# davnords/octic-vits

Measured on AMD Instinct MI355X. Metric: images/sec Hybrid Octic ViT-H/14 224² bf16 train step @1/2/4/8 MI355X, higher is better.
Workload: dtype bf16; 1 GPU; hybrid_deit_huge_patch14 (16 octic + 16 standard blocks, drop_path 0.5) DeiT-III train step: bf16-autocast fwd + bwd + LAMB + EMA, 224x224, batch 64/GPU (BASELINE configs[1]), data parallel over 1 GPU(s); global_batch=64, per_gpu_batch=64, accum_steps=1, parallelism=dp1, library_gemm_table=True, launch=hipGraph replay (whole step)

## Files before the change

include/octic_hip.h:

```cpp
#ifndef OCTIC_HIP_H
#define OCTIC_HIP_H

#include <stdint.h>

#ifdef __cplusplus
extern "C" {
#endif

#define OCTIC_ABI_VERSION 20

enum { OCTIC_F32 = 0, OCTIC_BF16 = 1, OCTIC_U8 = 2  };

enum {
  OCTIC_OK = 0,
  OCTIC_ESHAPE = -1,
  OCTIC_EALIGN = -2,
  OCTIC_EDTYPE = -3,
  OCTIC_ENULL = -4,
  OCTIC_EWORKSPACE = -5
};

typedef struct {
  void* ptr[5];
  int64_t ld[5];
// ... 47 lines not shown
  int c;
} octic_ln_finish_job;
int octic_layernorm_d8_bwd_finish_batch(const octic_ln_finish_job* jobs, int njobs, void* stream);

int octic_sample_blocks(const void* src, void* dst, const int64_t* idx, int64_t n, int64_t block_bytes, int scatter,
                        void* stream);

int octic_linear_d8_fwd(const octic_view* x, const void* const w[5], const float* bias, const octic_view* y,
                        const octic_view* resid, const float* rs, int64_t rows_per_sample,
                        const float* const cs[5], int64_t M, int cin, int cout, int dtype, int out_dtype,
                        void* stream);
int octic_linear_d8_fwd_skip(const octic_view* x, const void* const w[5], const float* bias, const octic_view* y,
                             const octic_view* resid, const float* rs, int64_t rows_per_sample,
                             const float* const cs[5], int64_t M, int cin, int cout, int dtype, int out_dtype,
                             const float* sample_scale, int64_t skip_rows_per_sample, void* stream);

int octic_linear_d8_prep(const float* const w32[5], const float* const cs[5], int cin, int cout, void* wb, void* wt,
                         int dtype, void* stream);
typedef struct octic_prep_item {
  const float* w[5];
  const float* cs[5];
  void* wb;
  void* wt;
  int32_t cin, cout;
  int32_t block_begin, block_count;
} octic_prep_item;
int octic_linear_d8_prep_batch_blocks(int cin, int cout);
int octic_linear_d8_prep_batch(const octic_prep_item* items_dev, int n_items, int total_blocks, int dtype, void* stream);

int octic_linear_d8_tile_n(int64_t M, int cin, int cout);
enum {
  OCTIC_LINEAR_WREG = 0,
  OCTIC_LINEAR_RING = 1,
  OCTIC_LINEAR_CLASSIC = 2
};
int octic_linear_d8_plan(int64_t M, int cin, int cout, int dtype, int out_dtype, int fused, int out[4]);
int octic_linear_d8_ring_order(int ngroups, const int* items, const int* ksteps, int slots_per_xcd, int* out_group,
                               int* out_item);

int octic_linear_d8_wgrad_has_colsum(int cin, int cout, int dtype);
enum {
  OCTIC_WGRAD_RING = 0,
  OCTIC_WGRAD_TILED = 1
};
int octic_linear_d8_wgrad_plan(int64_t M, int cin, int cout, int dtype, int out[4]);
int64_t octic_linear_d8_wgrad_workspace_bytes(int cin, int cout, int splits);
int octic_linear_d8_wgrad_splits(int64_t M, int cin, int cout);
int octic_linear_d8_wgrad_tile(int64_t M, int cin, int cout);
int octic_linear_d8_wgrad(const octic_view* x, const octic_view* dy, int64_t M, int cin, int cout, int dtype,
                          float* workspace, int splits, void* stream);
int octic_linear_d8_wgrad_finish(const float* workspace, int splits, int cin, int cout,
                                 const float* const w32[5], const float* const cs[5], const float* bias,
                                 const float* dysum, float* const dw[5], float* const dcs[5], float* dbias,
// ... 266 lines not shown
```

octic_vits_amd/_lib.py:

```python
import ctypes
import os
import re

HERE = os.path.dirname(os.path.abspath(__file__))
LIB_PATH = os.environ.get("OCTIC_LIB") or os.path.join(HERE, "liboctic_hip.so")
HEADER_PATH = os.path.join(HERE, "..", "include", "octic_hip.h")

F32, BF16, U8 = 0, 1, 2
ABI_VERSION = 20
(ROUTE_DENSE_TILE, ROUTE_DENSE_SPLIT, ROUTE_WGRAD_SLABS, ROUTE_WGRAD_TILE, ROUTE_LINEAR_RING, ROUTE_RING_EVEN,
 ROUTE_ATTN_LEGACY, ROUTE_ATTN_ONLINE, ROUTE_ATTN_BWD_PAIR, ROUTE_DENSE_IMAGE, ROUTE_DENSE_CLS2, ROUTE_ATTN_STREAM) = range(12)

(ATTN_FWD_PERSIST, ATTN_FWD_A80_ONESHOT, ATTN_FWD_A80_ONLINE, ATTN_FWD_RESIDENT, ATTN_FWD_STREAM, ATTN_FWD_F32) = range(6)
ATTN_BWD_SINGLE, ATTN_BWD_PAIR, ATTN_BWD_STREAM, ATTN_BWD_F32 = range(4)
LINEAR_WREG, LINEAR_RING, LINEAR_CLASSIC = range(3)
WGRAD_RING, WGRAD_TILED = range(2)

c_i64, c_int, c_float, c_void_p = ctypes.c_int64, ctypes.c_int, ctypes.c_float, ctypes.c_void_p
c_double = ctypes.c_double


class OcticView(ctypes.Structure):
    _fields_ = [("ptr", c_void_p * 5), ("ld", c_i64 * 5)]

# ... 9 lines not shown
    "octic_gelu_d8_bwd": (c_int, [VP, VP, VP, c_i64, c_int, c_int, c_void_p]),
    "octic_gelu_d8_fwd_skip": (c_int, [VP, VP, c_i64, c_int, c_int, c_void_p, c_i64, c_void_p]),
    "octic_gelu_d8_bwd_skip": (c_int, [VP, VP, VP, c_i64, c_int, c_int, c_void_p, c_i64, c_void_p]),
    "octic_layernorm_d8_fwd": (c_int, [VP, VP, c_void_p, c_void_p, c_void_p, c_i64, c_int, c_float, c_int, c_void_p]),
    "octic_layernorm_d8_bwd_blocks": (c_int, [c_i64]),
    "octic_layernorm_d8_bwd": (c_int, [VP, VP, c_void_p, c_void_p, VP, VP, c_void_p, c_i64, c_int, c_int, c_void_p]),
    "octic_layernorm_d8_bwd_cast": (c_int, [VP, VP, c_void_p, c_void_p, VP, VP, c_void_p, c_i64, c_int, c_void_p, c_i64,
                                            c_void_p, c_void_p]),
    "octic_layernorm_d8_bwd_finish": (c_int, [c_void_p, c_int, c_int, c_void_p, c_void_p, c_void_p]),
    "octic_layernorm_d8_bwd_finish_batch": (c_int, [c_void_p, c_int, c_void_p]),
    "octic_sample_blocks": (c_int, [c_void_p, c_void_p, c_void_p, c_i64, c_i64, c_int, c_void_p]),
    "octic_linear_d8_fwd": (c_int, [VP, c_void_p, c_void_p, VP, VP, c_void_p, c_i64, c_void_p, c_i64, c_int, c_int,
                                    c_int, c_int, c_void_p]),
    "octic_linear_d8_fwd_skip": (c_int, [VP, c_void_p, c_void_p, VP, VP, c_void_p, c_i64, c_void_p, c_i64, c_int, c_int,
                                         c_int, c_int, c_void_p, c_i64, c_void_p]),
    "octic_linear_d8_tile_n": (c_int, [c_i64, c_int, c_int]),
    "octic_linear_d8_plan": (c_int, [c_i64, c_int, c_int, c_int, c_int, c_int, ctypes.POINTER(c_int)]),
    "octic_linear_d8_ring_order": (c_int, [c_void_p, c_void_p, c_void_p, c_int, c_void_p, c_void_p]),
    "octic_linear_d8_wgrad_tile": (c_int, [c_i64, c_int, c_int]),
    "octic_linear_d8_wgrad_workspace_bytes": (c_i64, [c_int, c_int, c_int]),
    "octic_linear_d8_wgrad_splits": (c_int, [c_i64, c_int, c_int]),
    "octic_linear_d8_wgrad": (c_int, [VP, VP, c_i64, c_int, c_int, c_int, c_void_p, c_int, c_void_p]),
    "octic_linear_d8_wgrad_finish": (c_int, [c_void_p, c_int, c_int, c_int, c_void_p, c_void_p, c_void_p, c_void_p,
                                             c_void_p, c_void_p, c_void_p, c_void_p]),
    "octic_linear_d8_wgrad_finish_batch": (c_int, [c_void_p, c_int, c_void_p]),
    "octic_linear_d8_wgrad_has_colsum": (c_int, [c_int, c_int, c_int]),
    "octic_linear_d8_wgrad_plan": (c_int, [c_i64, c_int, c_int, c_int, ctypes.POINTER(c_int)]),
    "octic_lamb_workspace_floats": (c_i64, [c_int, c_int]),
    "octic_lamb_step": (c_int, [c_void_p] * 10 + [c_int, c_int, c_void_p, c_float, c_float, c_float, c_float, c_float,
                                                  c_int, c_float, c_void_p, c_void_p]),
    "octic_adamw_step": (c_int, [c_void_p] * 10 + [c_int, c_int, c_void_p, c_float, c_float, c_float, c_float, c_float,
                                                   c_int, c_float, c_void_p, c_void_p]),
    "octic_lamb_step_hp": (c_int, [c_void_p] * 10 + [c_int, c_int, c_void_p, c_void_p, c_float, c_float, c_float, c_float,
# ... 185 lines not shown
```

octic_vits_amd/csrc/gemm.hip:

```cpp
#include <stdlib.h>
#include <type_traits>
#include <mutex>
#include <vector>
#include "gemm_args.hpp"

namespace octic {

template <typename T> struct Elem;
template <> struct Elem<float> { static constexpr int EPC = 4; typedef f32x4 frag; };
template <> struct Elem<bf16> { static constexpr int EPC = 8; typedef bf16x8 frag; };

template <typename TOUT>
__device__ inline void store_out4(TOUT* p, f32x4 v);
template <>
__device__ inline void store_out4<float>(float* p, f32x4 v) { *(f32x4*)p = v; }
template <>
__device__ inline void store_out4<bf16>(bf16* p, f32x4 v) {
  bf16x4 o = {(bf16)v[0], (bf16)v[1], (bf16)v[2], (bf16)v[3]};
  *(bf16x4*)p = o;
}
template <typename TOUT>
__device__ inline f32x4 load_out4(const TOUT* p);
template <>
__device__ inline f32x4 load_out4<float>(const float* p) { return *(const f32x4*)p; }
// ... 287 lines not shown
    int r = tile - cum(k);
    bool found = false;
#pragma unroll
    for (int i = 0; i < 5; ++i) {
      const int s0 = (int)(((int64_t)k * T[i]) >> 3), sz = (int)(((int64_t)(k + 1) * T[i]) >> 3) - s0;
      if (!found && r < sz) {
        gi = i;
        lt = s0 + r;
        found = true;
      }
      if (!found) r -= sz;
    }
  }
}

template <typename TIN, typename TOUT, int EPI, int NT, int S, int BM = 128>
__global__ __launch_bounds__(BM * 2, 2) void linear_d8_ring_kernel(GemmArgs args) {
  constexpr int NW = BM / 32;
  constexpr int EPC = Elem<TIN>::EPC;
  constexpr int BKE = 8 * EPC;
  constexpr int MT = 2;
  constexpr int BN = 16 * NT;
  constexpr int STAGE = (BM + BN) * 128;
  constexpr int WI = BN / 8;
  constexpr int WQ = (WI + NW - 1) / NW;
  typedef typename Elem<TIN>::frag frag;
  extern __shared__ __attribute__((aligned(16))) char lds[];

  const int nwg = gridDim.x, bid = blockIdx.x;
  const int xcd = bid & 7, q8 = nwg >> 3, r8 = nwg & 7;
  const int tile = (xcd < r8 ? xcd * (q8 + 1) : r8 * (q8 + 1) + (xcd - r8) * q8) + (bid >> 3);
  (void)tile;
  int gi, lt;
  ring_item_of(args, nwg, bid, gi, lt);
  const GemmGroup& G = args.g[gi];
  const int mt = lt / G.n_chunks, nc = lt - mt * G.n_chunks;
  const int64_t m0 = (int64_t)mt * BM;
  const int nt_begin = nc * G.chunk;
  const int nt_count = (G.n_tiles - nt_begin) < G.chunk ? (G.n_tiles - nt_begin) : G.chunk;
  const int K = G.K, N = G.N;
  const int nkt = (K + BKE - 1) / BKE;
  const int steps = nt_count * nkt;
  const bool last_half_only = (K - (nkt - 1) * BKE) <= 4 * EPC;

  const int lane = threadIdx.x & 63;
  const int wid = __builtin_amdgcn_readfirstlane(threadIdx.x >> 6);
  const int fr = lane & 15, kg = lane >> 4;
  RTRACE(0);
#ifdef OCTIC_RING_TRACE
  {
    unsigned xcc, hwid;
    asm volatile("s_getreg_b32 %0, hwreg(HW_REG_XCC_ID)" : "=s"(xcc));
    asm volatile("s_getreg_b32 %0, hwreg(HW_REG_HW_ID)" : "=s"(hwid));
    if (tile < 2048 && lane == 0 && wid < 4) g_ring_trace[(tile * 4 + wid) * 64 + 63] = ((unsigned long long)hwid << 32) | xcc;
  }
#endif

  const int drow = lane >> 3;
  const int dkc = (lane & 7) ^ drow;
  const char* xsrc[4];
#pragma unroll
  for (int q = 0; q < 4; ++q) {
    int64_t mm = m0 + wid * 32 + q * 8 + drow;
    mm = mm < G.rows ? mm : G.rows - 1;
    const int64_t off = G.pair ? (mm >> 1) * G.a_ld + (mm & 1) * (int64_t)K : mm * G.a_ld;
    xsrc[q] = G.a + off * (int64_t)sizeof(TIN);
  }
  const int w_rem = WI % NW;
  const int w_cnt = WI / NW + (wid < w_rem ? 1 : 0);
  const int w_first = wid * (WI / NW) + (wid < w_rem ? wid : w_rem);
  const int dma_cnt = 4 + w_cnt;
// ... 325 lines not shown
    a.g[i].chunk = 1;
    a.g[i].n_chunks = a.g[i].n_tiles;
    a.g[i].tile_begin = t;
    t += a.g[i].n_chunks * a.g[i].m_tiles;
  }
  a.total_tiles = t;
  const size_t smem = (size_t)S * (BM + BN) * 128;
  {
    const int per_cu = (int)(160 * 1024 / smem) < 2 ? (int)(160 * 1024 / smem) : 2;
    plan_ring(a, t, device_cus() / 8 * (per_cu > 0 ? per_cu : 1));
  }
  static DeviceOnce once;
  if (once.first()) {
    (void)hipFuncSetAttribute((const void*)linear_d8_ring_kernel<TIN, TOUT, 0, NT, S, BM>, hipFuncAttributeMaxDynamicSharedMemorySize, (int)smem);
    (void)hipFuncSetAttribute((const void*)linear_d8_ring_kernel<TIN, TOUT, 1, NT, S, BM>, hipFuncAttributeMaxDynamicSharedMemorySize, (int)smem);
    (void)hipGetLastError();
  }
  if (fused) linear_d8_ring_kernel<TIN, TOUT, 1, NT, S, BM><<<t, BM * 2, smem, s>>>(a);
  else linear_d8_ring_kernel<TIN, TOUT, 0, NT, S, BM><<<t, BM * 2, smem, s>>>(a);
  return launch_status();
}

inline bool ring_ok(const GemmArgs& a, int dtype) {
  const int kstep = dtype == OCTIC_BF16 ? 32 : 16;
  for (int i = 0; i < a.ngroups; ++i)
    if (a.g[i].K % kstep) return false;
  return true;
}

inline bool ring_wide(const GemmArgs& a, int dtype) {
  bool ok = dtype == OCTIC_BF16 && a.lift_np == 0;
// ... 112 lines not shown
  for (int g = 0; g < ngroups; ++g) {
    a.g[g].K = ksteps[g] * 64;
    a.g[g].n_chunks = 1;
    a.g[g].chunk = 1;
    a.g[g].n_tiles = 1;
    a.g[g].m_tiles = items[g];
    a.g[g].tile_begin = t;
    t += items[g];
  }
  a.total_tiles = t;
  plan_ring(a, t, slots_per_xcd);
  for (int bid = 0; bid < t; ++bid) ring_item_of(a, t, bid, out_group[bid], out_item[bid]);
  return a.plan_mode;
}

extern "C" {

int octic_linear_d8_fwd_skip(const octic_view* x, const void* const w[5], const float* bias, const octic_view* y,
                             const octic_view* resid, const float* rs, int64_t rows_per_sample, const float* const cs[5],
                             int64_t M, int cin, int cout, int dtype, int out_dtype, const float* sample_scale,
                             int64_t skip_rows_per_sample, void* stream) {
  int e;
  if (sample_scale && (resid || rs || cs || skip_rows_per_sample <= 0 || M % skip_rows_per_sample != 0)) return OCTIC_ESHAPE;
  if ((e = check_c_dt(cin, dtype)) || (e = check_c_dt(cout, dtype)) || (e = check_c_dt(cout, out_dtype))) return e;
  if ((e = check_view(x, cin, dtype)) || (e = check_view(y, cout, out_dtype))) return e;
  if (resid && (e = check_view(resid, cout, out_dtype))) return e;
  if (!w) return OCTIC_ENULL;
  for (int i = 0; i < 5; ++i)
    if (!w[i] || (((uintptr_t)w[i]) & 15)) return w[i] ? OCTIC_EALIGN : OCTIC_ENULL;
  if (M <= 0 || (rs && rows_per_sample <= 0)) return OCTIC_ESHAPE;
  if (cs)
    for (int i = 0; i < 5; ++i)
      if (!cs[i]) return OCTIC_ENULL;
  GemmArgs a = {};
  a.rs = rs;
  a.rps = rs ? rows_per_sample : 1;
  a.skip = sample_scale;
  a.skip_rps = sample_scale ? skip_rows_per_sample : 1;
  d8_group_table(a, M, cin, cout);
  for (int gidx = 0; gidx < 5; ++gidx) {
    const int irrep = d8_group_irrep(gidx);
    GemmGroup& g = a.g[gidx];
    g.a = (const char*)x->ptr[irrep];
    g.a_ld = x->ld[irrep];
    g.w = (const char*)w[irrep];
    g.y = (char*)y->ptr[irrep];
    g.y_ld = y->ld[irrep];
    g.resid = resid ? (const char*)resid->ptr[irrep] : nullptr;
    g.r_ld = resid ? resid->ld[irrep] : 0;
    g.bias = (irrep == 0) ? bias : nullptr;
    g.cs = cs ? cs[irrep] : nullptr;
  }
  return dispatch_gemm(a, dtype, out_dtype, (hipStream_t)stream);
}

int octic_linear_d8_fwd(const octic_view* x, const void* const w[5], const float* bias, const octic_view* y,
                        const octic_view* resid, const float* rs, int64_t rows_per_sample, const float* const cs[5],
                        int64_t M, int cin, int cout, int dtype, int out_dtype, void* stream) {
  return octic_linear_d8_fwd_skip(x, w, bias, y, resid, rs, rows_per_sample, cs, M, cin, cout, dtype, out_dtype, nullptr, 0, stream);
}

int octic_linear_d8_plan(int64_t M, int cin, int cout, int dtype, int out_dtype, int fused, int out[4]) {
  if (!out) return OCTIC_ENULL;
  int e;
  if ((e = check_c_dt(cin, dtype)) || (e = check_c_dt(cout, dtype)) || (e = check_c_dt(cout, out_dtype))) return e;
  if (M <= 0) return OCTIC_ESHAPE;
  GemmArgs a = {};
  d8_group_table(a, M, cin, cout);
// ... 45 lines not shown
```

octic_vits_amd/csrc/gemm_args.hpp:

```cpp
#pragma once
#include "octic_common.hpp"

namespace octic {

struct GemmGroup {
  const char* a;
  int64_t a_ld;
  const char* w;
  char* y;
  int64_t y_ld;
  const char* resid;
  int64_t r_ld;
  const float* bias;
  const float* cs;
  int64_t rows;
  int K, N;
  int pair;
  int n_tiles, m_tiles;
  int chunk, n_chunks;
  int tile_begin;
  int wgs;
};

struct GemmArgs {
  GemmGroup g[5];
  int ngroups;
  int total_tiles;
  const float* rs;
  int64_t rps;
  int64_t lift_np;
  int lift_tok0;
  int plan_mode;
  int plan_nshort;
  int plan_a[8], plan_e[8];
  int plan_eb[8], plan_sb[8];
  const float* skip;
  int64_t skip_rps;
};

__device__ __forceinline__ unsigned lds_addr(const void* p) { return (unsigned)(uintptr_t)(__attribute__((address_space(3))) const char*)p; }
__device__ __forceinline__ bf16x8 lds_read16(unsigned addr) {
  bf16x8 v;
  asm volatile("ds_read_b128 %0, %1" : "=v"(v) : "v"(addr) : "memory");
  return v;
}
template <int N>
__device__ __forceinline__ void landed(bf16x8& v) {
  asm volatile("s_waitcnt lgkmcnt(%1)" : "+v"(v) : "n"(N) : "memory");
}

bool wreg_ok(const GemmArgs& a);
int launch_wreg(GemmArgs& a, int out_dtype, bool fused, hipStream_t s);
// ... 3 lines not shown
```

octic_vits_amd/d8_layers.py:

```python
import collections.abc
import math
from itertools import repeat

import torch
import torch.nn as nn
import torch.nn.functional as F

from . import functional as OF
from .d8_utils import SQRT2, SQRT2_OVER_4, convert_5tuple_to_8tuple, convert_8tuple_to_5tuple, expand_lift_kernel, packed_lift_weight
from .functional import Octic, as_packed, compute_dtype


def _ntuple(n):
    def parse(x):
        if isinstance(x, collections.abc.Iterable) and not isinstance(x, str):
            return tuple(x)
        return tuple(repeat(x, n))
    return parse


to_2tuple = _ntuple(2)

drop_path_mask_source = None

# ... 204 lines not shown
        if input_channels % 8 != 0 or output_channels % 8 != 0:
            raise ValueError()
        self.bias = bias
        self.input_channels, self.output_channels = input_channels, output_channels
        ci, co = input_channels // 8, output_channels // 8
        self.lin_A1 = nn.Linear(ci, co, bias=bias)
        self.lin_A2 = nn.Linear(ci, co, bias=False)
        self.lin_B1 = nn.Linear(ci, co, bias=False)
        self.lin_B2 = nn.Linear(ci, co, bias=False)
        self.lin_E = nn.Linear(2 * ci, 2 * co, bias=False)
        self._prep = OF.WeightPrep()

    def weights(self):
        return tuple(getattr(self, "lin_" + n).weight for n in _IRREPS)

    def forward(self, x_batched, resid=None, rs=None, cs=None, next_norm=None, skip_out=None, skip_dx=None):
        assert len(x_batched) == 5, "Input should be a 5-tuple"
        xp, cin = as_packed(x_batched)
        if 8 * cin != self.input_channels:
            raise ValueError(f"LinearD8: expected {self.input_channels} channels, got {8 * cin}")
        cout = self.output_channels // 8
        dtype = compute_dtype(xp)
        rps = xp.shape[-2] if xp.dim() >= 2 else 1
        if rs is not None and rs.numel() == xp.numel() // xp.shape[-1] and rs.numel() != xp.shape[0]:
            rps = 1
        cs5 = (None,) * 5 if cs is None else tuple(cs)
        if torch.compiler.is_compiling():
            from . import dispatch as _D
            xq = xp if xp.dtype == dtype else xp.to(dtype)
            fl = self._prep.flat if dtype == torch.bfloat16 else None
            pwb, pwt = fl if fl is not None else (None, None)
            y = torch.ops.octic.linear_d8(xq, *self.weights(), self.lin_A1.bias, resid, rs, *cs5, cin, cout, rps, pwb, pwt)
            return Octic(y, cout) if next_norm is None else (Octic(y, cout), None)
        if (next_norm is not None and resid is not None and OF.OCTIC_NEXT_NORM and xp.is_cuda and dtype == torch.bfloat16
                and resid.dtype == torch.float32 and type(next_norm) is LayerNormD8):
            a, beta = next_norm.affine()
            y, yn = OF.LinearD8NormFn.apply(xp, *self.weights(), self.lin_A1.bias, resid, rs, *cs5, cin, cout, rps, dtype,
                                            self._prep, *a, beta, next_norm.eps, skip_dx)
            return Octic(y, cout), Octic(yn, cout)
        y = OF.LinearD8Fn.apply(xp, *self.weights(), self.lin_A1.bias, resid, rs, *cs5, cin, cout, rps, dtype, self._prep,
                                skip_out, skip_dx)
        return Octic(y, cout) if next_norm is None else (Octic(y, cout), None)

    def extra_repr(self) -> str:
        return f"in_features={self.input_channels}, out_features={self.output_channels}, bias={self.bias is not None}"


class AffineD8(nn.Module):

    def __init__(self, dim, bias=True):
        super().__init__()
        if dim % 8 != 0:
            raise ValueError()
        self.alpha_A1 = nn.Parameter(torch.ones(dim // 8))
        self.alpha_A2 = nn.Parameter(torch.ones(dim // 8))
        self.alpha_B1 = nn.Parameter(torch.ones(dim // 8))
# ... 75 lines not shown
        self.fc2 = LinearD8(hidden_features, out_features, bias=bias[1])
        self.drop2 = DropoutD8(drop_probs[1])

    def _sample_mask(self, xs, resid, rs):
        if not (OF.LINEAR_SKIP_DROPPED and rs is not None and resid is not None and not COMPACT_DROP_PATH
                and type(self.fc1) is LinearD8 and type(self.fc2) is LinearD8 and type(self.act) is TritonGeluD8
                and type(self.norm) is nn.Identity and not self.drop1.active and not self.drop2.active
                and isinstance(xs, Octic) and xs.packed.dim() == 3 and xs.packed.is_cuda):
            return None
        xp = xs.packed
        return OF.linear_skip_scale(rs, xp.shape[1], xp.shape[0] * xp.shape[1])

    def forward(self, xs, resid=None, rs=None, cs=None, next_norm=None):
        mask = self._sample_mask(xs, resid, rs)
        if mask is not None:
            h = self.fc1(xs, skip_out=mask)
            a = Octic(OF.GeluD8PackedFn.apply(h.packed, h.c, mask, h.packed.shape[1]), h.c)
            return self.fc2(a, resid=resid, rs=rs, cs=cs, next_norm=next_norm, skip_dx=mask)
        xs = self.norm(self.drop1(self.act(self.fc1(xs))))
        if self.drop2.active or resid is None:
            out = _tail(self.drop2(self.fc2(xs)), resid, rs, cs)
            return out if next_norm is None else (out, None)
        return self.fc2(xs, resid=resid, rs=rs, cs=cs, next_norm=next_norm)


def _tail(ys, resid, rs, cs):
    if resid is None:
        return ys
    yp, c = as_packed(ys)
    yp = yp.to(resid.dtype)
    if cs is not None:
# ... 236 lines not shown
        if not OF.ops.attn_packed_ok(T, c, H, compute_dtype(xp)):
            return None
        if OF.skip_scale(rs, B) is None or OF.linear_skip_scale(rs, T, B * T) is None:
            return None
        if not OF.ops.attn_skips_dropped(B, T, 8 * (c // H), ld=(3 * 8 * c, 8 * c, 3 * 8 * c)):
            return None
        return rs

    def forward(self, xs, resid=None, rs=None, cs=None, next_norm=None):
        xp, c = as_packed(xs)
        if xp.dim() != 3:
            raise ValueError("AttentionD8 expects [B, N, C] irreps")
        drop = self.attn_drop.p if self.training else 0.
        rag = OF.RAGGED
        gemm_mask = self._gemm_mask(xp, c, resid, rs, drop, rag)
        qkv = self.qkv(xs if isinstance(xs, Octic) else Octic(xp, c), skip_out=gemm_mask)
        if rag is not None and rag.matches(xp):
            from . import ragged as _R
            if not (OF.ATTN_PACKED and drop == 0. and qkv.packed.is_cuda
                    and all(OF.ops.attn_packed_ok(T, c, self.num_heads, qkv.packed.dtype) for _, T, _ in rag.sets)):
                raise RuntimeError("AttentionD8: a ragged row tensor needs the packed attention kernels (bf16, head_dim 80 / 64)")
            on = Octic(_R.AttnPackedRaggedFn.apply(qkv.packed, rag, self.num_heads, c, (8 * c // self.num_heads) ** -0.5), c)
        elif (OF.ATTN_PACKED and drop == 0. and qkv.packed.is_cuda
                and OF.ops.attn_packed_ok(qkv.packed.shape[1], c, self.num_heads, qkv.packed.dtype)):
            if torch.compiler.is_compiling():
                from . import dispatch as _D
                on = Octic(torch.ops.octic.attn_packed(qkv.packed, self.num_heads, c, (8 * c // self.num_heads) ** -0.5)[0], c)
            else:
                on = Octic(OF.AttnPackedFn.apply(qkv.packed, self.num_heads, c, (8 * c // self.num_heads) ** -0.5,
                                                 None if (COMPACT_DROP_PATH or resid is None) else rs), c)
        else:
# ... 168 lines not shown
```

octic_vits_amd/functional.py:

```python
import os

import torch

from . import ops


class Octic(tuple):

    def __new__(cls, packed: torch.Tensor, c: int):
        self = super().__new__(cls, ops.split_packed(packed, c))
        self.packed, self.c = packed, c
        return self


def as_packed(xs):
    if isinstance(xs, Octic):
        return xs.packed, xs.c
    if len(xs) != 5:
        raise AssertionError("Input should be a 5-tuple")
    c = xs[0].shape[-1]
    if xs[4].shape[-2:] != (2, 2 * c):
        raise ValueError(f"E irrep must be [..., 2, {2 * c}], got {tuple(xs[4].shape)}")
    return torch.cat([xs[0], xs[1], xs[2], xs[3], xs[4].flatten(-2)], dim=-1), c

# ... 180 lines not shown
        return self.items is not None and self._current_ptrs() != self._ptrs

    def run(self):
        if self.items is None:
            return
        ops.check(ops.lib().octic_linear_d8_prep_batch(ops._p(self.items), len(self.preps), self.total_blocks,
                                                       ops.dt_code(torch.bfloat16), ops._stream(self.items)))
        for p, (wb, wt), flat in zip(self.preps, self.bufs, self.flats):
            p.adopt(wb, wt, flat)


class LinearD8Fn(torch.autograd.Function):

    @staticmethod
    def forward(ctx, x, wA1, wA2, wB1, wB2, wE, bias, resid, rs, sA1, sA2, sB1, sB2, sE, cin, cout, rps, dtype, prep,
                skip_out=None, skip_dx=None):
        w5 = (wA1, wA2, wB1, wB2, wE)
        cs5 = None if sA1 is None else (sA1, sA2, sB1, sB2, sE)
        ops._require_cuda(x)
        fused = resid is not None
        out_dtype = resid.dtype if fused else dtype
        x_in_dtype = x.dtype
        if x.dtype != dtype:
            x = ops.cast_rowscale(_c(x.float()), None, 1, dtype, cin)
        x = _c(x)
        wb, wt = prep.get(w5, cs5, dtype, cin, cout)
        lead = x.shape[:-1]
        M = x.numel() // (8 * cin)
        y = torch.empty(lead + (8 * cout,), dtype=out_dtype, device=x.device)
        b32 = None if bias is None else _c(bias.detach().float())
        cs32 = None if cs5 is None else [_c(s.detach().float()) for s in cs5]
        rs32 = None if rs is None else _c(rs.float())
        rv = ops.pview(_c(resid), cout) if fused else None
        plain = not fused and rs32 is None and cs32 is None
        ss_out = linear_skip_scale(skip_out, rps, M) if plain else None
        ops.linear_fwd(ops.pview(x, cin), wb, b32, ops.pview(y, cout), M, cin, cout, dtype, out_dtype, x,
                       resid_v=rv, rs=rs32, rps=rps, cs5=cs32, sample_scale=ss_out, skip_rps=rps)
        ctx.save_for_backward(x, rs32, b32, linear_skip_scale(skip_dx, rps, M), *w5, *(cs32 or []))
        ctx.meta = (cin, cout, rps, dtype, fused, cs5 is not None, bias is not None, x_in_dtype, wt)
        return y

    @staticmethod
    def backward(ctx, dy):
        cin, cout, rps, dtype, fused, has_cs, has_bias, x_in_dtype, wt = ctx.meta
        x, rs32, b32, ss_dx, *rest = ctx.saved_tensors
        w5, cs32 = rest[:5], (rest[5:] if has_cs else None)
        M = x.numel() // (8 * cin)
        dy = _c(dy)
        if fused or rs32 is not None or dy.dtype != dtype:
            g = ops.cast_rowscale(_c(dy.float()), rs32, rps, dtype, cout)
        else:
            g = dy
        gv, xv = ops.pview(g, cout), ops.pview(x, cin)
        dx = None
        if ctx.needs_input_grad[0]:
            dx = torch.empty(x.shape, dtype=dtype, device=x.device)
            ops.linear_fwd(gv, wt, None, ops.pview(dx, cin), M, cout, cin, dtype, dtype, x, sample_scale=ss_dx, skip_rps=rps)
            if dx.dtype != x_in_dtype:
                dx = dx.to(x_in_dtype)
        dysum = ops.colsum_a1(gv, M, cout, dtype, x) if (has_bias and not ops.wgrad_has_colsum(cin, cout, dtype)) else None
        w32 = [_c(w.detach().float()) for w in w5] if has_cs else None
        f32_masters = all(w.dtype == torch.float32 for w in w5)
        dw, dcs, dbias = ops.linear_wgrad(xv, gv, M, cin, cout, dtype, x, w32=w32, cs5=cs32, bias=b32, dysum=dysum,
                                          want_bias=has_bias, may_defer=f32_masters, wparams=w5 if f32_masters else None)
        if not f32_masters:
            dw = [d.to(w.dtype) for d, w in zip(dw, w5)]
        dcs = dcs if has_cs else [None] * 5
        return (dx, *dw, dbias, dy if fused else None, None, *dcs, None, None, None, None, None, None, None)


class LinearD8NormFn(torch.autograd.Function):

    @staticmethod
    def forward(ctx, x, wA1, wA2, wB1, wB2, wE, bias, resid, rs, sA1, sA2, sB1, sB2, sE, cin, cout, rps, dtype, prep,
                a1, a2, b1, b2, ae, beta, eps, skip_dx=None):
        w5 = (wA1, wA2, wB1, wB2, wE)
        cs5 = None if sA1 is None else (sA1, sA2, sB1, sB2, sE)
        ops._require_cuda(x)
        x_in_dtype = x.dtype
        if x.dtype != dtype:
            x = ops.cast_rowscale(_c(x.float()), None, 1, dtype, cin)
        x = _c(x)
        wb, wt = prep.get(w5, cs5, dtype, cin, cout)
        M = x.numel() // (8 * cin)
        y = torch.empty(x.shape[:-1] + (8 * cout,), dtype=resid.dtype, device=x.device)
        b32 = None if bias is None else _c(bias.detach().float())
        cs32 = None if cs5 is None else [_c(s.detach().float()) for s in cs5]
        rs32 = None if rs is None else _c(rs.float())
        ops.linear_fwd(ops.pview(x, cin), wb, b32, ops.pview(y, cout), M, cin, cout, dtype, resid.dtype, x,
                       resid_v=ops.pview(_c(resid), cout), rs=rs32, rps=rps, cs5=cs32)
        alpha = None if a1 is None else [_c(t.float()) for t in (a1, a2, b1, b2, ae)]
        yn, stats = ops.layernorm_fwd(y, alpha, None if beta is None else _c(beta.float()), eps, dtype, cout)
        ctx.save_for_backward(x, rs32, b32, y, stats, linear_skip_scale(skip_dx, rps, M), *w5, *(cs32 or []), *(alpha or []))
        ctx.meta = (cin, cout, rps, dtype, cs5 is not None, bias is not None, x_in_dtype, wt, alpha is not None,
                    beta is not None)
        ctx.set_materialize_grads(False)
        return y, yn

    @staticmethod
    def backward(ctx, dy, dyn):
        cin, cout, rps, dtype, has_cs, has_bias, x_in_dtype, wt, has_affine, has_beta = ctx.meta
        x, rs32, b32, y, stats, ss_dx, *rest = ctx.saved_tensors
        w5 = rest[:5]
        cs32 = rest[5:10] if has_cs else None
        alpha = rest[(10 if has_cs else 5):] if has_affine else None
# ... 106 lines not shown

def _linear_skip_from_env():
    return os.environ.get("OCTIC_LINEAR_SKIP", "1").strip() != "0"


LINEAR_SKIP_DROPPED = _linear_skip_from_env()


def linear_skip_scale(rs, rps, M, rows_to=None):
    if (not LINEAR_SKIP_DROPPED or rs is None or rows_to is not None or torch.compiler.is_compiling() or not rs.is_cuda
            or rs.dtype != torch.float32 or rs.dim() != 1 or not rs.is_contiguous() or rps < 2 or rs.numel() * rps != M):
        return None
    return rs.detach()


class AttnPackedFn(torch.autograd.Function):

    @staticmethod
    def forward(ctx, qkv, H, c, scale, sample_scale=None):
        qkv = _c(qkv)
        ss = skip_scale(sample_scale, qkv.shape[0])
        o, lse = ops.attn_fwd_packed(qkv, H, c, scale, sample_scale=ss)
        ctx.save_for_backward(qkv, o, lse, ss)
        ctx.meta = (H, c, scale)
        return o

    @staticmethod
    def backward(ctx, do):
        qkv, o, lse, ss = ctx.saved_tensors
        H, c, scale = ctx.meta
# ... 639 lines not shown
```

octic_vits_amd/ops.py:

```python
import ctypes
import operator

import torch

from . import _lib
from ._lib import BF16, F32, OcticView, PtrArray5, check, lib

_DT = {torch.float32: F32, torch.bfloat16: BF16}
_DTN = {torch.float32: "f32", torch.bfloat16: "bf16"}


class KernelTimer:

    def __init__(self):
        self.on = False
        self.records = []
        self.overhead_us = 0.0

    def enable(self):
        self.on, self.records = True, []
        pairs = []
        for _ in range(64):
            e0, e1 = torch.cuda.Event(enable_timing=True), torch.cuda.Event(enable_timing=True)
            e0.record()
# ... 337 lines not shown
    ws = _DW_WS.get(dy0.device)
    if ws is None or ws.numel() < need:
        ws = _DW_WS[dy0.device] = torch.zeros(need, dtype=torch.uint8, device=dy0.device)
    if dw0 is None:
        dw0 = torch.empty((N0, K), dtype=torch.float32, device=dy0.device)
    if dw1 is None:
        dw1 = torch.empty((N1, K), dtype=torch.float32, device=dy0.device)
    t = KERNEL_TIMER.start()
    check(lib().octic_dense_wgrad_tn_pair_skip(_p(dy0), _p(x0), N0, dy0.stride(0), x0.stride(0), _p(dw0), _p(dy1), _p(x1), N1,
                                               dy1.stride(0), x1.stride(0), _p(dw1), M, K, _p(ss), rps, _p(ws), _stream(dy0)))
    KERNEL_TIMER.stop(t, f"dense_tn_kernel<{N0}+{N1}x{K}>", 2 * M * (N0 + N1 + 2 * K) + 4 * (N0 + N1) * K, 2.0 * M * (N0 + N1) * K)
    return dw0, dw1


def linear_fwd(xv, w5, bias, yv, M, cin, cout, dtype, out_dtype, ref, resid_v=None, rs=None, rps=1, cs5=None, sample_scale=None,
               skip_rps=0):
    ss, srps = _row_sample_scale(sample_scale, skip_rps, M, ref, "linear_fwd")
    t = KERNEL_TIMER.start()
    check(lib().octic_linear_d8_fwd_skip(ctypes.byref(xv), _arr5(w5), _p(bias), ctypes.byref(yv),
                                         ctypes.byref(resid_v) if resid_v is not None else None, _p(rs), int(rps),
                                         _arr5(cs5) if cs5 is not None else None, M, cin, cout, dt_code(dtype),
                                         dt_code(out_dtype), _p(ss), srps, _stream(ref)))
    if t is not None:
        es, eo = (2 if dtype == torch.bfloat16 else 4), (2 if out_dtype == torch.bfloat16 else 4)
        nbytes = M * 8 * cin * es + M * 8 * cout * eo * (2 if resid_v is not None else 1) + 8 * cin * cout * es
        fused = int(resid_v is not None or rs is not None or cs5 is not None)
        KERNEL_TIMER.stop(t, linear_kernel_name(cin, cout, dtype, out_dtype, fused, M), nbytes, 24.0 * M * cin * cout)


def linear_kernel_name(cin, cout, dtype, out_dtype, fused, M):
    kernel, _, fused, _ = _lib.plan("octic_linear_d8_plan", M, cin, cout, dt_code(dtype), dt_code(out_dtype), int(fused))
    if kernel == _lib.LINEAR_WREG:
        return f"linear_d8_wreg_kernel<{_DTN[out_dtype]},{fused}>"
    if kernel == _lib.LINEAR_RING:
        return f"linear_d8_ring_kernel<{_DTN[dtype]},{_DTN[out_dtype]},{fused}>"
    return f"linear_d8_kernel<{_DTN[dtype]},{_DTN[out_dtype]}>"

# ... 968 lines not shown
```

Measured before the change: 1157 images/s.

## Skip GEMM tiles for drop-path-dropped samples in octic ring linear kernel

Adds a SKIP variant of the ring linear kernel. Each workgroup builds a live/dead bitmap of M-tiles from the per-sample drop-path scale and remaps its work items so that live tiles are scheduled first. Dead tiles only copy the residual, or write zeros, instead of running the full GEMM. This is wired into fused residual projections and into the dx backward GEMMs of fc1 and qkv, and it is on by default through OCTIC_RING_SKIP. The goal is to avoid the matmul work that drop_path 0.5 throws away, in exchange for a bitmap-build prologue in every workgroup and more complex scheduling.

Result: faster. 1169 images/s, median of 6 (+1.1%).

```diff
diff --git a/include/octic_hip.h b/include/octic_hip.h
--- a/include/octic_hip.h
+++ b/include/octic_hip.h
@@ -85,6 +85,10 @@
                              const octic_view* resid, const float* rs, int64_t rows_per_sample,
                              const float* const cs[5], int64_t M, int cin, int cout, int dtype, int out_dtype,
                              const float* sample_scale, int64_t skip_rows_per_sample, void* stream);
+int octic_linear_d8_fwd_dropped(const octic_view* x, const void* const w[5], const float* bias, const octic_view* y,
+                                const octic_view* resid, const float* rs, int64_t rows_per_sample,
+                                const float* const cs[5], int64_t M, int cin, int cout, int dtype, int out_dtype,
+                                const float* dropped, int64_t dropped_rows_per_sample, void* stream);
 
 int octic_linear_d8_prep(const float* const w32[5], const float* const cs[5], int cin, int cout, void* wb, void* wt,
                          int dtype, void* stream);
@@ -108,6 +112,9 @@
 int octic_linear_d8_plan(int64_t M, int cin, int cout, int dtype, int out_dtype, int fused, int out[4]);
 int octic_linear_d8_ring_order(int ngroups, const int* items, const int* ksteps, int slots_per_xcd, int* out_group,
                                int* out_item);
+int octic_linear_d8_ring_order_dropped(int ngroups, const int* items, const int* ksteps, int slots_per_xcd, const int* n_chunks,
+                                       const unsigned char* dead_long, const unsigned char* dead_short, int* out_group,
+                                       int* out_item, int* out_dead);
 
 int octic_linear_d8_wgrad_has_colsum(int cin, int cout, int dtype);
 enum {
diff --git a/octic_vits_amd/_lib.py b/octic_vits_amd/_lib.py
--- a/octic_vits_amd/_lib.py
+++ b/octic_vits_amd/_lib.py
@@ -47,9 +47,13 @@
                                     c_int, c_int, c_void_p]),
     "octic_linear_d8_fwd_skip": (c_int, [VP, c_void_p, c_void_p, VP, VP, c_void_p, c_i64, c_void_p, c_i64, c_int, c_int,
                                          c_int, c_int, c_void_p, c_i64, c_void_p]),
+    "octic_linear_d8_fwd_dropped": (c_int, [VP, c_void_p, c_void_p, VP, VP, c_void_p, c_i64, c_void_p, c_i64, c_int, c_int,
+                                            c_int, c_int, c_void_p, c_i64, c_void_p]),
     "octic_linear_d8_tile_n": (c_int, [c_i64, c_int, c_int]),
     "octic_linear_d8_plan": (c_int, [c_i64, c_int, c_int, c_int, c_int, c_int, ctypes.POINTER(c_int)]),
     "octic_linear_d8_ring_order": (c_int, [c_void_p, c_void_p, c_void_p, c_int, c_void_p, c_void_p]),
+    "octic_linear_d8_ring_order_dropped": (c_int, [c_int, c_void_p, c_void_p, c_int, c_void_p, c_void_p, c_void_p, c_void_p,
+                                                   c_void_p, c_void_p]),
     "octic_linear_d8_wgrad_tile": (c_int, [c_i64, c_int, c_int]),
     "octic_linear_d8_wgrad_workspace_bytes": (c_i64, [c_int, c_int, c_int]),
     "octic_linear_d8_wgrad_splits": (c_int, [c_i64, c_int, c_int]),
diff --git a/octic_vits_amd/csrc/gemm.hip b/octic_vits_amd/csrc/gemm.hip
--- a/octic_vits_amd/csrc/gemm.hip
+++ b/octic_vits_amd/csrc/gemm.hip
@@ -325,7 +325,94 @@
   }
 }
 
-template <typename TIN, typename TOUT, int EPI, int NT, int S, int BM = 128>
+constexpr int kRingMaskCap = 1024;
+constexpr int kRingMaskWords = kRingMaskCap / 64;
+
+__host__ __device__ inline int bm_count(const unsigned long long* bm, int words) {
+  int c = 0;
+  for (int i = 0; i < words; ++i) c += __builtin_popcountll(bm[i]);
+  return c;
+}
+__host__ __device__ inline int bm_select(const unsigned long long* bm, int words, int r, bool set) {
+  for (int i = 0; i < words; ++i) {
+    unsigned long long w = set ? bm[i] : ~bm[i];
+    const int c = __builtin_popcountll(w);
+    if (r < c || i == words - 1) {
+      int pos = 0;
+#pragma unroll
+      for (int sh = 32; sh; sh >>= 1) {
+        const unsigned long long lo = w & ((1ull << sh) - 1);
+        const int cl = __builtin_popcountll(lo);
+        if (r >= cl) {
+          r -= cl;
+          w >>= sh;
+          pos += sh;
+        } else {
+          w = lo;
+        }
+      }
+      return i * 64 + pos;
+    }
+    r -= c;
+  }
+  return 0;
+}
+
+__host__ __device__ inline void ring_item_masked(const GemmArgs& args, int nwg, int bid, const unsigned long long* live_long,
+                                                 const unsigned long long* live_short, int& gi, int& lt, bool& dead) {
+  const int ML = args.g[0].m_tiles, NC0 = args.g[0].n_chunks, MS = args.g[1].m_tiles, NCS = args.g[1].n_chunks;
+  const int nshort = args.ngroups - 1;
+  const int wl = (ML + 63) >> 6, ws = (MS + 63) >> 6;
+  const int LL = bm_count(live_long, wl), LS = bm_count(live_short, ws);
+  const int x = bid & 7, l = bid >> 3;
+  int f;
+  if (((ML + 7) >> 3) * NC0 <= (nwg >> 3)) {
+    const int c0 = LL >> 3, R = LL & 7;
+    if (l < (c0 + (x < R ? 1 : 0)) * NC0) {
+      const int q = l / NC0;
+      gi = 0;
+      lt = bm_select(live_long, wl, q * 8 + x, true) * NC0 + (l - q * NC0);
+      dead = false;
+      return;
+    }
+    f = l < (c0 + 1) * NC0 ? (l - c0 * NC0) * (8 - R) + (x - R) : NC0 * (8 - R) + (l - (c0 + 1) * NC0) * 8 + x;
+  } else {
+    if (bid < LL * NC0) {
+      const int q = bid / NC0;
+      gi = 0;
+      lt = bm_select(live_long, wl, q, true) * NC0 + (bid - q * NC0);
+      dead = false;
+      return;
+    }
+    f = bid - LL * NC0;
+  }
+  const int per_tile = NCS * nshort;
+  dead = f >= LS * per_tile;
+  if (dead) f -= LS * per_tile;
+  if (dead && f < (ML - LL) * NC0) {
+    const int q = f / NC0;
+    gi = 0;
+    lt = bm_select(live_long, wl, q, false) * NC0 + (f - q * NC0);
+    return;
+  }
+  if (dead) f -= (ML - LL) * NC0;
+  const int q = f / per_tile, r = f - q * per_tile, g = r / NCS;
+  gi = 1 + g;
+  lt = bm_select(live_short, ws, q, !dead) * NCS + (r - g * NCS);
+}
+
+inline bool ring_mask_ok(const GemmArgs& a) {
+  if (a.ngroups < 2 || a.lift_np > 0 || a.dropped_rps <= 0) return false;
+  if (a.g[0].m_tiles > kRingMaskCap || a.g[1].m_tiles > kRingMaskCap || a.g[0].rows >= (1ll << 31) - 256) return false;
+  for (int g = 1; g < a.ngroups; ++g) {
+    if (a.g[g].chunk != 1 || a.g[g].m_tiles != a.g[1].m_tiles || a.g[g].n_chunks != a.g[1].n_chunks || a.g[g].rows != a.g[1].rows ||
+        a.g[g].pair != a.g[1].pair)
+      return false;
+  }
+  return a.g[0].chunk == 1;
+}
+
+template <typename TIN, typename TOUT, int EPI, int NT, int S, int BM = 128, bool SKIP = false>
 __global__ __launch_bounds__(BM * 2, 2) void linear_d8_ring_kernel(GemmArgs args) {
   constexpr int NW = BM / 32;
   constexpr int EPC = Elem<TIN>::EPC;
@@ -343,7 +430,35 @@
   const int tile = (xcd < r8 ? xcd * (q8 + 1) : r8 * (q8 + 1) + (xcd - r8) * q8) + (bid >> 3);
   (void)tile;
   int gi, lt;
-  ring_item_of(args, nwg, bid, gi, lt);
+  bool dead_item = false;
+  if constexpr (SKIP) {
+    __shared__ unsigned long long live_bm[2 * kRingMaskWords];
+    const int lane0 = threadIdx.x & 63, wid0 = __builtin_amdgcn_readfirstlane(threadIdx.x >> 6);
+    const int wl = (args.g[0].m_tiles + 63) >> 6, ws = (args.g[1].m_tiles + 63) >> 6;
+    const float* dropped = args.dropped;
+    const unsigned rps = (unsigned)args.dropped_rps;
+    for (int w = wid0; w < wl + ws; w += BM / 32) {
+      const bool lg = w < wl;
+      const unsigned rows = (unsigned)(lg ? args.g[0].rows : args.g[1].rows);
+      const int psh = lg ? args.g[0].pair : args.g[1].pair;
+      const unsigned r0 = (unsigned)(((lg ? w : w - wl) << 6) + lane0) * (unsigned)BM;
+      bool live = false;
+      if (r0 < rows) {
+        const unsigned r1 = r0 + BM - 1 < rows ? r0 + BM - 1 : rows - 1;
+        const unsigned b1 = (r1 >> psh) / rps;
+        for (unsigned b = (r0 >> psh) / rps; b <= b1; ++b) live = live || dropped[b] != 0.0f;
+      }
+      const unsigned long long m = __ballot(live);
+      if (lane0 == 0) live_bm[lg ? w : kRingMaskWords + (w - wl)] = m;
+    }
+    __syncthreads();
+    ring_item_masked(args, nwg, bid, live_bm, live_bm + kRingMaskWords, gi, lt, dead_item);
+    gi = __builtin_amdgcn_readfirstlane(gi);
+    lt = __builtin_amdgcn_readfirstlane(lt);
+    dead_item = __builtin_amdgcn_readfirstlane((int)dead_item) != 0;
+  } else {
+    ring_item_of(args, nwg, bid, gi, lt);
+  }
   const GemmGroup& G = args.g[gi];
   const int mt = lt / G.n_chunks, nc = lt - mt * G.n_chunks;
   const int64_t m0 = (int64_t)mt * BM;
@@ -366,6 +481,31 @@
     if (tile < 2048 && lane == 0 && wid < 4) g_ring_trace[(tile * 4 + wid) * 64 + 63] = ((unsigned long long)hwid << 32) | xcc;
   }
 #endif
+
+  if constexpr (SKIP) {
+    if (dead_item) {
+      constexpr int OPC = 16 / (int)sizeof(TOUT), CPR = BN / OPC;
+      typedef typename std::conditional<sizeof(TOUT) == 4, f32x4, bf16x8>::type piece_t;
+      const int nb = nt_begin * BN;
+      const int pshift = G.pair ? 1 : 0;
+      const int64_t rows = G.rows, y_ld = G.y_ld, r_ld = G.r_ld;
+      TOUT* const yb = (TOUT*)G.y;
+      const TOUT* const rb = (const TOUT*)G.resid;
+#pragma unroll 4
+      for (int p = threadIdx.x; p < BM * CPR; p += BM * 2) {
+        const int r = p / CPR, c = p - r * CPR;
+        const int64_t mm = m0 + r;
+        const int n = nb + c * OPC;
+        if (mm < rows && n < N) {
+          const int64_t tok = mm >> pshift, half = mm & pshift;
+          piece_t v = {};
+          if constexpr (EPI == 1) v = *(const piece_t*)(rb + tok * r_ld + half * N + n);
+          *(piece_t*)(yb + tok * y_ld + half * N + n) = v;
+        }
+      }
+      return;
+    }
+  }
 
   const int drow = lane >> 3;
   const int dkc = (lane & 7) ^ drow;
@@ -721,7 +861,18 @@
   if (once.first()) {
     (void)hipFuncSetAttribute((const void*)linear_d8_ring_kernel<TIN, TOUT, 0, NT, S, BM>, hipFuncAttributeMaxDynamicSharedMemorySize, (int)smem);
     (void)hipFuncSetAttribute((const void*)linear_d8_ring_kernel<TIN, TOUT, 1, NT, S, BM>, hipFuncAttributeMaxDynamicSharedMemorySize, (int)smem);
+    if constexpr (std::is_same<TIN, bf16>::value) {
+      (void)hipFuncSetAttribute((const void*)linear_d8_ring_kernel<TIN, TOUT, 0, NT, S, BM, true>, hipFuncAttributeMaxDynamicSharedMemorySize, (int)smem);
+      (void)hipFuncSetAttribute((const void*)linear_d8_ring_kernel<TIN, TOUT, 1, NT, S, BM, true>, hipFuncAttributeMaxDynamicSharedMemorySize, (int)smem);
+    }
     (void)hipGetLastError();
+  }
+  if constexpr (std::is_same<TIN, bf16>::value) {
+    if (a.dropped && ring_mask_ok(a)) {
+      if (fused) linear_d8_ring_kernel<TIN, TOUT, 1, NT, S, BM, true><<<t, BM * 2, smem, s>>>(a);
+      else linear_d8_ring_kernel<TIN, TOUT, 0, NT, S, BM, true><<<t, BM * 2, smem, s>>>(a);
+      return launch_status();
+    }
   }
   if (fused) linear_d8_ring_kernel<TIN, TOUT, 1, NT, S, BM><<<t, BM * 2, smem, s>>>(a);
   else linear_d8_ring_kernel<TIN, TOUT, 0, NT, S, BM><<<t, BM * 2, smem, s>>>(a);
@@ -864,13 +1015,53 @@
   return a.plan_mode;
 }
 
+extern "C" int octic_linear_d8_ring_order_dropped(int ngroups, const int* items, const int* ksteps, int slots_per_xcd, const int* n_chunks,
+                                            const unsigned char* dead_long, const unsigned char* dead_short, int* out_group,
+                                            int* out_item, int* out_dead) {
+  if (ngroups < 1 || ngroups > 5 || !items || !ksteps || !dead_long || !dead_short || !out_group || !out_item) return OCTIC_ENULL;
+  (void)slots_per_xcd;
+  GemmArgs a = {};
+  a.ngroups = ngroups;
+  a.dropped_rps = 1;
+  int t = 0;
+  for (int g = 0; g < ngroups; ++g) {
+    if (items[g] <= 0 || (n_chunks && n_chunks[g] <= 0)) return OCTIC_ESHAPE;
+    a.g[g].K = ksteps[g] * 64;
+    a.g[g].n_chunks = n_chunks ? n_chunks[g] : 1;
+    a.g[g].chunk = 1;
+    a.g[g].n_tiles = a.g[g].n_chunks;
+    a.g[g].m_tiles = items[g];
+    a.g[g].rows = (int64_t)items[g] * kBM;
+    a.g[g].tile_begin = t;
+    t += items[g] * a.g[g].n_chunks;
+  }
+  a.total_tiles = t;
+  if (!ring_mask_ok(a)) return OCTIC_ESHAPE;
+  unsigned long long bm[2 * kRingMaskWords] = {};
+  for (int i = 0; i < items[0]; ++i)
+    if (!dead_long[i]) bm[i >> 6] |= 1ull << (i & 63);
+  for (int i = 0; i < items[1]; ++i)
+    if (!dead_short[i]) bm[kRingMaskWords + (i >> 6)] |= 1ull << (i & 63);
+  for (int bid = 0; bid < t; ++bid) {
+    bool dead = false;
+    ring_item_masked(a, t, bid, bm, bm + kRingMaskWords, out_group[bid], out_item[bid], dead);
+    if (out_dead) out_dead[bid] = dead ? 1 : 0;
+  }
+  return t;
+}
+
 extern "C" {
 
-int octic_linear_d8_fwd_skip(const octic_view* x, const void* const w[5], const float* bias, const octic_view* y,
-                             const octic_view* resid, const float* rs, int64_t rows_per_sample, const float* const cs[5],
-                             int64_t M, int cin, int cout, int dtype, int out_dtype, const float* sample_scale,
-                             int64_t skip_rows_per_sample, void* stream) {
+static int linear_d8_launch(const octic_view* x, const void* const w[5], const float* bias, const octic_view* y,
+                            const octic_view* resid, const float* rs, int64_t rows_per_sample, const float* const cs[5],
+                            int64_t M, int cin, int cout, int dtype, int out_dtype, const float* sample_scale,
+                            int64_t skip_rows_per_sample, const float* dropped, int64_t dropped_rows_per_sample, void* stream) {
   int e;
+  if (dropped) {
+    if (dropped_rows_per_sample <= 0 || dropped_rows_per_sample >= (1ll << 31) || M % dropped_rows_per_sample != 0) return OCTIC_ESHAPE;
+    const bool plain = !resid && !rs && !cs;
+    if (plain ? bias != nullptr : (!resid || !rs || dropped_rows_per_sample != rows_per_sample)) return OCTIC_ESHAPE;
+  }
   if (sample_scale && (resid || rs || cs || skip_rows_per_sample <= 0 || M % skip_rows_per_sample != 0)) return OCTIC_ESHAPE;
   if ((e = check_c_dt(cin, dtype)) || (e = check_c_dt(cout, dtype)) || (e = check_c_dt(cout, out_dtype))) return e;
   if ((e = check_view(x, cin, dtype)) || (e = check_view(y, cout, out_dtype))) return e;
@@ -887,6 +1078,8 @@
   a.rps = rs ? rows_per_sample : 1;
   a.skip = sample_scale;
   a.skip_rps = sample_scale ? skip_rows_per_sample : 1;
+  a.dropped = dropped;
+  a.dropped_rps = dropped ? (int)dropped_rows_per_sample : 0;
   d8_group_table(a, M, cin, cout);
   for (int gidx = 0; gidx < 5; ++gidx) {
     const int irrep = d8_group_irrep(gidx);
@@ -901,7 +1094,24 @@
     g.bias = (irrep == 0) ? bias : nullptr;
     g.cs = cs ? cs[irrep] : nullptr;
   }
+  if (a.dropped && a.lift_np > 0) return OCTIC_ESHAPE;
   return dispatch_gemm(a, dtype, out_dtype, (hipStream_t)stream);
+}
+
+int octic_linear_d8_fwd_skip(const octic_view* x, const void* const w[5], const float* bias, const octic_view* y,
+                             const octic_view* resid, const float* rs, int64_t rows_per_sample, const float* const cs[5],
+                             int64_t M, int cin, int cout, int dtype, int out_dtype, const float* sample_scale,
+                             int64_t skip_rows_per_sample, void* stream) {
+  return linear_d8_launch(x, w, bias, y, resid, rs, rows_per_sample, cs, M, cin, cout, dtype, out_dtype, sample_scale,
+                          skip_rows_per_sample, nullptr, 0, stream);
+}
+
+int octic_linear_d8_fwd_dropped(const octic_view* x, const void* const w[5], const float* bias, const octic_view* y,
+                                const octic_view* resid, const float* rs, int64_t rows_per_sample, const float* const cs[5],
+                                int64_t M, int cin, int cout, int dtype, int out_dtype, const float* dropped,
+                                int64_t dropped_rows_per_sample, void* stream) {
+  return linear_d8_launch(x, w, bias, y, resid, rs, rows_per_sample, cs, M, cin, cout, dtype, out_dtype, nullptr, 0, dropped,
+                          dropped_rows_per_sample, stream);
 }
 
 int octic_linear_d8_fwd(const octic_view* x, const void* const w[5], const float* bias, const octic_view* y,
diff --git a/octic_vits_amd/csrc/gemm_args.hpp b/octic_vits_amd/csrc/gemm_args.hpp
--- a/octic_vits_amd/csrc/gemm_args.hpp
+++ b/octic_vits_amd/csrc/gemm_args.hpp
@@ -36,6 +36,8 @@
   int plan_eb[8], plan_sb[8];
   const float* skip;
   int64_t skip_rps;
+  const float* dropped;
+  int dropped_rps;
 };
 
 __device__ __forceinline__ unsigned lds_addr(const void* p) { return (unsigned)(uintptr_t)(__attribute__((address_space(3))) const char*)p; }
diff --git a/octic_vits_amd/d8_layers.py b/octic_vits_amd/d8_layers.py
--- a/octic_vits_amd/d8_layers.py
+++ b/octic_vits_amd/d8_layers.py
@@ -242,7 +242,7 @@
     def weights(self):
         return tuple(getattr(self, "lin_" + n).weight for n in _IRREPS)
 
-    def forward(self, x_batched, resid=None, rs=None, cs=None, next_norm=None, skip_out=None, skip_dx=None):
+    def forward(self, x_batched, resid=None, rs=None, cs=None, next_norm=None, skip_out=None, skip_dx=None, zero_dx=None):
         assert len(x_batched) == 5, "Input should be a 5-tuple"
         xp, cin = as_packed(x_batched)
         if 8 * cin != self.input_channels:
@@ -267,7 +267,7 @@
                                             self._prep, *a, beta, next_norm.eps, skip_dx)
             return Octic(y, cout), Octic(yn, cout)
         y = OF.LinearD8Fn.apply(xp, *self.weights(), self.lin_A1.bias, resid, rs, *cs5, cin, cout, rps, dtype, self._prep,
-                                skip_out, skip_dx)
+                                skip_out, skip_dx, zero_dx)
         return Octic(y, cout) if next_norm is None else (Octic(y, cout), None)
 
     def extra_repr(self) -> str:
@@ -373,7 +373,7 @@
     def forward(self, xs, resid=None, rs=None, cs=None, next_norm=None):
         mask = self._sample_mask(xs, resid, rs)
         if mask is not None:
-            h = self.fc1(xs, skip_out=mask)
+            h = self.fc1(xs, skip_out=mask, zero_dx=mask)
             a = Octic(OF.GeluD8PackedFn.apply(h.packed, h.c, mask, h.packed.shape[1]), h.c)
             return self.fc2(a, resid=resid, rs=rs, cs=cs, next_norm=next_norm, skip_dx=mask)
         xs = self.norm(self.drop1(self.act(self.fc1(xs))))
@@ -640,7 +640,11 @@
         drop = self.attn_drop.p if self.training else 0.
         rag = OF.RAGGED
         gemm_mask = self._gemm_mask(xp, c, resid, rs, drop, rag)
-        qkv = self.qkv(xs if isinstance(xs, Octic) else Octic(xp, c), skip_out=gemm_mask)
+        zero_dx = rs if (rs is not None and resid is not None and not COMPACT_DROP_PATH and not (rag is not None and rag.matches(xp))
+                         and OF.ATTN_PACKED and drop == 0. and xp.is_cuda and not torch.compiler.is_compiling()
+                         and not self.proj_drop.active and type(self.qkv) is LinearD8 and type(self.proj) is LinearD8
+                         and OF.ops.attn_packed_ok(xp.shape[1], c, self.num_heads, compute_dtype(xp))) else None
+        qkv = self.qkv(xs if isinstance(xs, Octic) else Octic(xp, c), skip_out=gemm_mask, zero_dx=zero_dx)
         if rag is not None and rag.matches(xp):
             from . import ragged as _R
             if not (OF.ATTN_PACKED and drop == 0. and qkv.packed.is_cuda
diff --git a/octic_vits_amd/functional.py b/octic_vits_amd/functional.py
--- a/octic_vits_amd/functional.py
+++ b/octic_vits_amd/functional.py
@@ -218,7 +218,7 @@
 
     @staticmethod
     def forward(ctx, x, wA1, wA2, wB1, wB2, wE, bias, resid, rs, sA1, sA2, sB1, sB2, sE, cin, cout, rps, dtype, prep,
-                skip_out=None, skip_dx=None):
+                skip_out=None, skip_dx=None, zero_dx=None):
         w5 = (wA1, wA2, wB1, wB2, wE)
         cs5 = None if sA1 is None else (sA1, sA2, sB1, sB2, sE)
         ops._require_cuda(x)
@@ -238,16 +238,19 @@
         rv = ops.pview(_c(resid), cout) if fused else None
         plain = not fused and rs32 is None and cs32 is None
         ss_out = linear_skip_scale(skip_out, rps, M) if plain else None
+        dropped = ring_skip_scale(rs32, rps, M) if fused else None
         ops.linear_fwd(ops.pview(x, cin), wb, b32, ops.pview(y, cout), M, cin, cout, dtype, out_dtype, x,
-                       resid_v=rv, rs=rs32, rps=rps, cs5=cs32, sample_scale=ss_out, skip_rps=rps)
-        ctx.save_for_backward(x, rs32, b32, linear_skip_scale(skip_dx, rps, M), *w5, *(cs32 or []))
+                       resid_v=rv, rs=rs32, rps=rps, cs5=cs32, sample_scale=ss_out, skip_rps=rps, dropped=dropped, dropped_rps=rps)
+        ss_dx = linear_skip_scale(skip_dx, rps, M)
+        z_dx = ring_skip_scale(zero_dx, rps, M) if (plain and ss_dx is None) else None
+        ctx.save_for_backward(x, rs32, b32, ss_dx, z_dx, *w5, *(cs32 or []))
         ctx.meta = (cin, cout, rps, dtype, fused, cs5 is not None, bias is not None, x_in_dtype, wt)
         return y
 
     @staticmethod
     def backward(ctx, dy):
         cin, cout, rps, dtype, fused, has_cs, has_bias, x_in_dtype, wt = ctx.meta
-        x, rs32, b32, ss_dx, *rest = ctx.saved_tensors
+        x, rs32, b32, ss_dx, z_dx, *rest = ctx.saved_tensors
         w5, cs32 = rest[:5], (rest[5:] if has_cs else None)
         M = x.numel() // (8 * cin)
         dy = _c(dy)
@@ -259,7 +262,8 @@
         dx = None
         if ctx.needs_input_grad[0]:
             dx = torch.empty(x.shape, dtype=dtype, device=x.device)
-            ops.linear_fwd(gv, wt, None, ops.pview(dx, cin), M, cout, cin, dtype, dtype, x, sample_scale=ss_dx, skip_rps=rps)
+            ops.linear_fwd(gv, wt, None, ops.pview(dx, cin), M, cout, cin, dtype, dtype, x, sample_scale=ss_dx, skip_rps=rps,
+                           dropped=z_dx, dropped_rps=rps)
             if dx.dtype != x_in_dtype:
                 dx = dx.to(x_in_dtype)
         dysum = ops.colsum_a1(gv, M, cout, dtype, x) if (has_bias and not ops.wgrad_has_colsum(cin, cout, dtype)) else None
@@ -270,7 +274,7 @@
         if not f32_masters:
             dw = [d.to(w.dtype) for d, w in zip(dw, w5)]
         dcs = dcs if has_cs else [None] * 5
-        return (dx, *dw, dbias, dy if fused else None, None, *dcs, None, None, None, None, None, None, None)
+        return (dx, *dw, dbias, dy if fused else None, None, *dcs, None, None, None, None, None, None, None, None)
 
 
 class LinearD8NormFn(torch.autograd.Function):
@@ -292,7 +296,8 @@
         cs32 = None if cs5 is None else [_c(s.detach().float()) for s in cs5]
         rs32 = None if rs is None else _c(rs.float())
         ops.linear_fwd(ops.pview(x, cin), wb, b32, ops.pview(y, cout), M, cin, cout, dtype, resid.dtype, x,
-                       resid_v=ops.pview(_c(resid), cout), rs=rs32, rps=rps, cs5=cs32)
+                       resid_v=ops.pview(_c(resid), cout), rs=rs32, rps=rps, cs5=cs32, dropped=ring_skip_scale(rs32, rps, M),
+                       dropped_rps=rps)
         alpha = None if a1 is None else [_c(t.float()) for t in (a1, a2, b1, b2, ae)]
         yn, stats = ops.layernorm_fwd(y, alpha, None if beta is None else _c(beta.float()), eps, dtype, cout)
         ctx.save_for_backward(x, rs32, b32, y, stats, linear_skip_scale(skip_dx, rps, M), *w5, *(cs32 or []), *(alpha or []))
@@ -429,6 +434,17 @@
     return rs.detach()
 
 
+def _ring_skip_from_env():
+    return os.environ.get("OCTIC_RING_SKIP", "1").strip() != "0"
+
+
+RING_SKIP_DROPPED = _ring_skip_from_env()
+
+
+def ring_skip_scale(rs, rps, M):
+    return linear_skip_scale(rs, rps, M) if RING_SKIP_DROPPED else None
+
+
 class AttnPackedFn(torch.autograd.Function):
 
     @staticmethod
diff --git a/octic_vits_amd/ops.py b/octic_vits_amd/ops.py
--- a/octic_vits_amd/ops.py
+++ b/octic_vits_amd/ops.py
@@ -375,13 +375,17 @@
 
 
 def linear_fwd(xv, w5, bias, yv, M, cin, cout, dtype, out_dtype, ref, resid_v=None, rs=None, rps=1, cs5=None, sample_scale=None,
-               skip_rps=0):
+               skip_rps=0, dropped=None, dropped_rps=0):
     ss, srps = _row_sample_scale(sample_scale, skip_rps, M, ref, "linear_fwd")
-    t = KERNEL_TIMER.start()
-    check(lib().octic_linear_d8_fwd_skip(ctypes.byref(xv), _arr5(w5), _p(bias), ctypes.byref(yv),
-                                         ctypes.byref(resid_v) if resid_v is not None else None, _p(rs), int(rps),
-                                         _arr5(cs5) if cs5 is not None else None, M, cin, cout, dt_code(dtype),
-                                         dt_code(out_dtype), _p(ss), srps, _stream(ref)))
+    dr, drps = _row_sample_scale(dropped, dropped_rps, M, ref, "linear_fwd")
+    if ss is not None and dr is not None:
+        raise ValueError("linear_fwd: sample_scale and dropped are two contracts for one mask - pass one of them")
+    t = KERNEL_TIMER.start()
+    entry = lib().octic_linear_d8_fwd_skip if dr is None else lib().octic_linear_d8_fwd_dropped
+    check(entry(ctypes.byref(xv), _arr5(w5), _p(bias), ctypes.byref(yv),
+                ctypes.byref(resid_v) if resid_v is not None else None, _p(rs), int(rps),
+                _arr5(cs5) if cs5 is not None else None, M, cin, cout, dt_code(dtype),
+                dt_code(out_dtype), _p(ss if dr is None else dr), srps if dr is None else drps, _stream(ref)))
     if t is not None:
         es, eo = (2 if dtype == torch.bfloat16 else 4), (2 if out_dtype == torch.bfloat16 else 4)
         nbytes = M * 8 * cin * es + M * 8 * cout * eo * (2 if resid_v is not None else 1) + 8 * cin * cout * es
```
